# cosmicBboy/movenet

Measured on AMD Instinct MI355X. Metric: autoregressive audio samples/sec (16 kHz, 30-layer WaveNet, whole job), higher is better.
Workload: dtype f32

## Files before the change

movenet_amd/csrc/generate_fold.hip:

```cpp
#include <cstdlib>
#include <type_traits>

#include "common.h"
#include "gen_common.h"
#include "pipe_common.h"

namespace mvn {

namespace fold {
constexpr int C = 64, Q = 256, NT = 512, LPS = 3;
constexpr int KQ = 4, KPER = 16, NF4 = 4;
constexpr int MAT_F = 2 * C * C;
enum { M_A0 = 0, M_A0P, M_A1, M_A2, M_B2P,
       M_B1, M_B1P, M_B2, M_RR, M_RS,
       M_WP0, M_WP1, M_WP2, M_SS,
       N_MAT };
constexpr int N_LDS_MAT = 4;
constexpr int V_CB1 = 0, V_CB2 = 2 * C, V_BSP = 4 * C, V_BR0 = 5 * C, V_BS0 = 6 * C, V_BR1 = 7 * C,
              V_BS1 = 8 * C, V_BR2 = 9 * C, VEC_F = 10 * C;
constexpr int STAGE_F = N_MAT * MAT_F + VEC_F;
constexpr int CTX_LAYER_F = MAT_F + 2 * C;
constexpr int EMB_F = 2 * Q * C;
constexpr int W1_F = Q * C, W2_F = Q * Q, WSL_F = C * C;
constexpr int HEAD_F = W1_F + Q + W2_F + Q + WSL_F + C;
// ... 15 lines not shown
    m.w[2 * i + 1] = v2f{v.z, v.w};
  }
}
__device__ __forceinline__ v2f pk_fma_hi(v2f w, v2f xpair, v2f acc) {
  asm("v_pk_fma_f32 %0, %1, %2, %0 op_sel:[0,1,0]" : "+v"(acc) : "v"(w), "v"(xpair));
  return acc;
}
__device__ __forceinline__ v2f pk_mul_hi(v2f w, v2f xpair) {
  v2f r;
  asm("v_pk_mul_f32 %0, %1, %2 op_sel:[0,1]" : "=v"(r) : "v"(w), "v"(xpair));
  return r;
}
template <bool INIT>
__device__ __forceinline__ void pair_acc(v2f (&acc)[4], const v2f (&w)[16], const f4 (&x)[4]) {
#pragma unroll
  for (int i = 0; i < 4; ++i) {
    if (INIT && i == 0) {
      acc[0] = w[0] * v2f{x[0].x, x[0].x};
      acc[1] = w[1] * v2f{x[0].y, x[0].y};
      acc[2] = w[2] * v2f{x[0].z, x[0].z};
      acc[3] = pk_mul_hi(w[3], v2f{x[0].z, x[0].w});
    } else {
      acc[0] = __builtin_elementwise_fma(w[4 * i], v2f{x[i].x, x[i].x}, acc[0]);
      acc[1] = __builtin_elementwise_fma(w[4 * i + 1], v2f{x[i].y, x[i].y}, acc[1]);
      acc[2] = __builtin_elementwise_fma(w[4 * i + 2], v2f{x[i].z, x[i].z}, acc[2]);
      acc[3] = pk_fma_hi(w[4 * i + 3], v2f{x[i].z, x[i].w}, acc[3]);
    }
  }
}
__device__ __forceinline__ v2f pair_sum(const v2f (&acc)[4]) { return (acc[0] + acc[2]) + (acc[1] + acc[3]); }
template <int H>
__device__ __forceinline__ float split_dot(const v2f (&w)[16], const f4 (&x)[4]) {
  v2f a0 = w[8 * H] * v2f{x[0].x, x[0].y}, a1 = w[8 * H + 1] * v2f{x[0].z, x[0].w};
  v2f a2 = w[8 * H + 2] * v2f{x[1].x, x[1].y}, a3 = w[8 * H + 3] * v2f{x[1].z, x[1].w};
  a0 = __builtin_elementwise_fma(w[8 * H + 4], v2f{x[2].x, x[2].y}, a0);
  a1 = __builtin_elementwise_fma(w[8 * H + 5], v2f{x[2].z, x[2].w}, a1);
  a2 = __builtin_elementwise_fma(w[8 * H + 6], v2f{x[3].x, x[3].y}, a2);
  a3 = __builtin_elementwise_fma(w[8 * H + 7], v2f{x[3].z, x[3].w}, a3);
  const v2f t = (a0 + a2) + (a1 + a3);
  return t.x + t.y;
}

typedef __attribute__((address_space(3))) float lds_f;
typedef float vf4 __attribute__((ext_vector_type(4)));
typedef __attribute__((address_space(3))) vf4 lds_f4;
__device__ __forceinline__ f4 lds_load4(unsigned addr) {
  const vf4 v = *(const lds_f4 *)(uintptr_t)addr;
  f4 r;
  r.x = v.x; r.y = v.y; r.z = v.z; r.w = v.w;
  return r;
}
__device__ __forceinline__ unsigned lds_addr(const float *p) { return (unsigned)(uintptr_t)(lds_f *)p; }
#define LDSF(addr, off) (*(lds_f *)(uintptr_t)((addr) + 4u * (unsigned)(off)))
template <int N4>
__device__ __forceinline__ void ldsv(f4 (&x)[N4], unsigned addr, int off) {
#pragma unroll
  for (int i = 0; i < N4; ++i) x[i] = lds_load4(addr + 4u * (unsigned)off + 16u * i);
}

__device__ __forceinline__ v2f pair_dot_lds(unsigned waddr, unsigned xaddr) {
  v2f acc[4];
#pragma unroll
  for (int i = 0; i < 4; ++i) {
    const f4 wa = lds_load4(waddr + 4096u * (2 * i)), wb = lds_load4(waddr + 4096u * (2 * i + 1));
    const f4 x = lds_load4(xaddr + 16u * i);
    if (i == 0) {
      acc[0] = v2f{wa.x, wa.y} * v2f{x.x, x.x};
      acc[1] = v2f{wa.z, wa.w} * v2f{x.y, x.y};
      acc[2] = v2f{wb.x, wb.y} * v2f{x.z, x.z};
      acc[3] = pk_mul_hi(v2f{wb.z, wb.w}, v2f{x.z, x.w});
    } else {
      acc[0] = __builtin_elementwise_fma(v2f{wa.x, wa.y}, v2f{x.x, x.x}, acc[0]);
      acc[1] = __builtin_elementwise_fma(v2f{wa.z, wa.w}, v2f{x.y, x.y}, acc[1]);
      acc[2] = __builtin_elementwise_fma(v2f{wb.x, wb.y}, v2f{x.z, x.z}, acc[2]);
      acc[3] = pk_fma_hi(v2f{wb.z, wb.w}, v2f{x.z, x.w}, acc[3]);
    }
  }
  return pair_sum(acc);
}
template <int H>
__device__ __forceinline__ float split_dot_lds(unsigned waddr, unsigned xaddr) {
  f4 w[4], x[4];
#pragma unroll
  for (int i = 0; i < 4; ++i) {
    w[i] = lds_load4(waddr + 4096u * (4 * H + i));
    x[i] = lds_load4(xaddr + 16u * i);
  }
  v2f a0 = v2f{w[0].x, w[0].y} * v2f{x[0].x, x[0].y}, a1 = v2f{w[0].z, w[0].w} * v2f{x[0].z, x[0].w};
  v2f a2 = v2f{w[1].x, w[1].y} * v2f{x[1].x, x[1].y}, a3 = v2f{w[1].z, w[1].w} * v2f{x[1].z, x[1].w};
  a0 = __builtin_elementwise_fma(v2f{w[2].x, w[2].y}, v2f{x[2].x, x[2].y}, a0);
  a1 = __builtin_elementwise_fma(v2f{w[2].z, w[2].w}, v2f{x[2].z, x[2].w}, a1);
  a2 = __builtin_elementwise_fma(v2f{w[3].x, w[3].y}, v2f{x[3].x, x[3].y}, a2);
  a3 = __builtin_elementwise_fma(v2f{w[3].z, w[3].w}, v2f{x[3].z, x[3].w}, a3);
  const v2f t = (a0 + a2) + (a1 + a3);
  return t.x + t.y;
}

template <bool MULTI>
__global__ __launch_bounds__(512, 2) void gen_fold_kernel(GenArgs a, u64 *hand, unsigned *err, int NS, int nb, int nseq) {
  using namespace fold;
  extern __shared__ __attribute__((aligned(16))) float smem[];
  const int tid = threadIdx.x, lane = tid & 63, wave = tid >> 6;
  const int xcd = blockIdx.x & 7, slot = blockIdx.x >> 3;
  const int in_xcd = (PIPE_XCD_CUS / NS) * NS;
  int b, s;
  if (slot < in_xcd) {
    b = xcd + 8 * (slot / NS);
    s = slot % NS;
  } else {
    const int idx = xcd * (PIPE_XCD_CUS - in_xcd) + (slot - in_xcd);
    b = 8 * (PIPE_XCD_CUS / NS) + idx / NS;
    s = idx % NS;
  }
  if (b >= nb) return;
  if (__hip_atomic_load(err, __ATOMIC_RELAXED, __HIP_MEMORY_SCOPE_AGENT) != 0) return;
  const int L = a.L;
  const int s_next = s + 1 == NS ? 0 : s + 1;
  const int G = MULTI ? (nseq - b + nb - 1) / nb : 1;
  int bq = b;
  u64 *inbox = hand + ((size_t)b * NS + s) * GRAN;
  u64 *outbox = hand + ((size_t)b * NS + s_next) * GRAN;
  int *iflag = (int *)(smem + LDS_FLOATS - 16);
  float *pfs = smem + LDS_FLOATS;
  const bool fast_edge = pipe_edge_is_fast(err + 16, b, s, s_next, NS, iflag);

  auto layer_stage = [&](auto first_stage) {
    constexpr bool FIRST = decltype(first_stage)::value;
    const bool last = s == NS - 2;
    const int l0 = s * LPS, nl = min(LPS, L - l0);
    const bool chain = tid < 256;
    const int t = tid & 255, c = t >> 2, kq = t & 3;
    const bool lead = kq == 0;
    float *lmat = smem;
    constexpr int O_XP = 0;
    constexpr int O_ZL = C;
    constexpr int O_Z0 = 2 * C, O_Z1 = 3 * C;
    constexpr int O_X0 = 4 * C;
    constexpr int O_B1 = 5 * C, O_B2 = 7 * C;
    constexpr int O_PAST = 9 * C;
    constexpr int O_CTX = 12 * C;
    constexpr int O_VEC = 13 * C;
    float *vec = smem + N_LDS_MAT * MAT_F;
    unsigned vc = lds_addr(vec) + 4u * c;
    unsigned vq = lds_addr(vec) + 4u * KPER * kq;
    asm volatile("" : "+v"(vc), "+v"(vq));
    u64 *ob = outbox + c;
    const u64 *ibs = inbox + 2 * C + c;
    float *ring = a.state + (size_t)b * a.state_per_seq;
    auto bind = [&](int g) {
      bq = b + g * nb;
      inbox = hand + ((size_t)bq * NS + s) * GRAN;
      outbox = hand + ((size_t)bq * NS + s_next) * GRAN;
      ob = outbox + c;
      ibs = inbox + 2 * C + c;
      ring = a.state + (size_t)bq * a.state_per_seq;
    };
    const float *sec = a.w + EMB_F + (size_t)s * STAGE_F;
    const float *vecs = sec + N_MAT * MAT_F;

    FoldMat m0, m1 = {}, m2, m3, m4;
    {
      const int first = chain ? M_A0 : M_B1;
      fold_load(m0, sec + (size_t)(first + 0) * MAT_F, t);
      if (!FIRST) fold_load(m1, sec + (size_t)(first + 1) * MAT_F, t);
      fold_load(m2, sec + (size_t)(first + 2) * MAT_F, t);
      fold_load(m3, sec + (size_t)(first + 3) * MAT_F, t);
      fold_load(m4, sec + (size_t)(first + 4) * MAT_F, t);
      const f4 *src = (const f4 *)(sec + (size_t)M_WP0 * MAT_F);
      for (int i = tid; i < N_LDS_MAT * MAT_F / 4; i += NT) ((f4 *)lmat)[i] = src[i];
    }
    float pf[LPS], pg[LPS];
    float (&xs)[LPS] = pf;
    int doff[LPS], dmask[LPS];
    for (int i = tid; i < VEC_F; i += NT) vec[O_VEC + i] = vecs[i];
#pragma unroll
    for (int j = 0; j < LPS; ++j) {
      pf[j] = 0.f; pg[j] = 0.f;
      const int l = l0 + j;
      dmask[j] = j < nl ? (1 << (l % a.layer_size)) - 1 : 0;
      doff[j] = j < nl ? ring_offset(l, a.layer_size, C) : 0;
    }

    float popv[LPS] = {0.f, 0.f, 0.f};
    auto prefetch_pops = [&](int tn) {
      if (MULTI && !chain && lead) {
        int cq = c;
        asm volatile("" : "+v"(cq));
#pragma unroll
        for (int j = 0; j < LPS; ++j)
          if (j < nl) popv[j] = ring_load(ring + doff[j] + cq + (tn & dmask[j]) * C);
      }
    };
    auto precompute = [&](int tn, bool push, bool popped) {
      int tq = t;
      asm volatile("" : "+v"(tq));
      const int cq = tq >> 2, kk = tq & 3;
      if (!chain && lead) {
#pragma unroll
        for (int j = 0; j < LPS; ++j)
          if (j < nl) {
            float *base = ring + doff[j] + cq;
            if (push) base[((tn - 1) & dmask[j]) * C] = xs[j];
            const float pv = (push && dmask[j] == 0) ? xs[j]
                             : (MULTI && popped) ? popv[j] : ring_load(base + (tn & dmask[j]) * C);
            vec[O_PAST + j * C + cq] = pv;
          }
      }
      if (a.ctx_tm && chain && tq < C) vec[O_CTX + tq] = a.ctx_tm[(size_t)bq * a.ctx_stride_b + (size_t)tn * C + tq];
      __syncthreads();
      if (chain) {
        const unsigned wm = lds_addr(lmat) + 16u * tq, xq = lds_addr(vec) + 4u * (O_PAST + KPER * kk);
        const v2f p0 = pair_dot_lds(wm, xq);
        const v2f p1 = pair_dot_lds(wm + 4u * MAT_F, xq + 4u * C);
        const v2f p2 = pair_dot_lds(wm + 8u * MAT_F, xq + 8u * C);
        pf[0] = chan_sum<KQ>(p0.x);
        pg[0] = chan_sum<KQ>(p0.y);
        pf[1] = chan_sum<KQ>(p1.x) + vec[O_VEC + V_CB1 + cq];
        pg[1] = chan_sum<KQ>(p1.y) + vec[O_VEC + V_CB1 + C + cq];
        pf[2] = chan_sum<KQ>(p2.x) + vec[O_VEC + V_CB2 + cq];
        pg[2] = chan_sum<KQ>(p2.y) + vec[O_VEC + V_CB2 + C + cq];
        if (a.ctx_tm) {
#pragma unroll
          for (int j = 0; j < LPS; ++j)
            if (j < nl) {
              const float *wc = a.wctx + (size_t)(l0 + j) * CTX_LAYER_F;
              pf[j] += chan_sum<KQ>(dot_stream<NF4>((const f4 *)wc, 256, tq, vec + O_CTX + KPER * kk)) + wc[MAT_F + cq];
              pg[j] += chan_sum<KQ>(dot_stream<NF4>((const f4 *)wc + NF4 * 256, 256, tq, vec + O_CTX + KPER * kk)) +
// ... 1 lines not shown
            }
        }
      }
    };
    auto save_pf = [&](int g) {
      if (MULTI && chain && lead) {
        float *q = pfs + ((size_t)g * C + c) * PFS_F;
        *(f4 *)q = f4{pf[0], pg[0], pf[1], pg[1]};
        *(v2f *)(q + 4) = v2f{pf[2], pg[2]};
      }
    };
    auto load_pf = [&](int g) {
      if (MULTI && chain) {
        const float *q = pfs + ((size_t)g * C + c) * PFS_F;
        const f4 v = *(const f4 *)q;
        const v2f w = *(const v2f *)(q + 4);
        pf[0] = v.x; pg[0] = v.y; pf[1] = v.z; pg[1] = v.w; pf[2] = w.x; pg[2] = w.y;
      }
    };
    __syncthreads();
    if (MULTI) {
      for (int g = 0; g < G; ++g) {
        bind(g);
        precompute(a.t_begin, false, false);
        save_pf(g);
        __syncthreads();
      }
    } else {
      precompute(a.t_begin, false, false);
    }

    bool alive = true;
    for (int ts = a.t_begin; ts < a.t_end && alive; ++ts)
    for (int g = 0; g < G; ++g) {
      if (MULTI) {
        bind(g);
        if (ts + 1 < a.t_end) prefetch_pops(ts + 1);
      }
      const unsigned epoch = (unsigned)(ts - a.t_begin + 1);
      if (wave == 0) {
        float v[2];
        const bool ok = FIRST ? wait_inbox64(inbox, epoch, err, v) : wait_inbox<2>(inbox, epoch, err, v);
        if (ok && (!FIRST || lane < 32)) {
          float *dst = vec + 2 * lane;
          dst[0] = v[0];
          dst[1] = v[1];
        }
        if (lane == 0) iflag[0] = ok ? 1 : 0;
      }
      lds_barrier();
      MVN_STAMP(b, s, ts - a.t_begin, 0);
      load_pf(g);
      float xv = 0.f;
      MVN_FINE(b, s, ts - a.t_begin, 0, 0);
      if (chain) {
        f4 xa[NF4], xb[NF4];
        ldsv<NF4>(xa, vq, O_XP);
        if (!FIRST) ldsv<NF4>(xb, vq, O_ZL);
        v2f acc[4];
        pair_acc<true>(acc, m0.w, xa);
        if (!FIRST) pair_acc<false>(acc, m1.w, xb);
        const v2f fg = pair_sum(acc);
        const float f = chan_sum<KQ>(fg.x) + pf[0];
        const float g = chan_sum<KQ>(fg.y) + pg[0];
        const float z = gate_fast(f, g);
        if (lead) LDSF(vc, O_Z0) = z;
        MVN_FINE(b, s, ts - a.t_begin, 1, 0);
      } else {
        f4 xa[NF4], xb[NF4];
        ldsv<NF4>(xa, vq, O_XP);
        if (!FIRST) ldsv<NF4>(xb, vq, O_ZL);
        v2f acc[4];
        pair_acc<true>(acc, m0.w, xa);
        if (!FIRST) pair_acc<false>(acc, m1.w, xb);
        const v2f fg = pair_sum(acc);
        float r = 0.f;
        if (!FIRST) r = split_dot<0>(m3.w, xb);
        const float f = chan_sum<KQ>(fg.x);
        const float g = chan_sum<KQ>(fg.y);
        if (!FIRST) r = chan_sum<KQ>(r);
        if (lead) {
          xv = LDSF(vc, O_XP) + r;
          LDSF(vc, O_X0) = xv;
          xs[0] = xv;
          LDSF(vc, O_B1) = f;
          LDSF(vc, O_B1 + C) = g;
        }
        MVN_FINE(b, s, ts - a.t_begin, 6, 256);
      }
      lds_barrier();
      MVN_FINE(b, s, ts - a.t_begin, 2, 0);
      v2f b2 = {0.f, 0.f};
      if (chain) {
        f4 xz[NF4];
        ldsv<NF4>(xz, vq, O_Z0);
        v2f acc[4], acc2[4];
        pair_acc<true>(acc, m2.w, xz);
        pair_acc<true>(acc2, m4.w, xz);
        const v2f fg = pair_sum(acc);
        b2 = pair_sum(acc2);
        asm volatile("" : "+v"(b2));
        const float f = chan_sum<KQ>(fg.x) + (LDSF(vc, O_B1) + pf[1]);
        const float g = chan_sum<KQ>(fg.y) + (LDSF(vc, O_B1 + C) + pg[1]);
        const float z = gate_fast(f, g);
        if (lead) LDSF(vc, O_Z1) = z;
        MVN_FINE(b, s, ts - a.t_begin, 3, 0);
      } else {
        f4 xa[NF4];
        ldsv<NF4>(xa, vq, O_X0);
        v2f acc[4];
        pair_acc<true>(acc, m2.w, xa);
        const v2f fg = pair_sum(acc);
        const float f = chan_sum<KQ>(fg.x);
        const float g = chan_sum<KQ>(fg.y);
        if (lead) {
          LDSF(vc, O_B2) = f;
          LDSF(vc, O_B2 + C) = g;
        }
        MVN_FINE(b, s, ts - a.t_begin, 7, 256);
      }
      lds_barrier();
      MVN_FINE(b, s, ts - a.t_begin, 4, 0);
      if (chain) {
        f4 xz[NF4];
        ldsv<NF4>(xz, vq, O_Z1);
        v2f acc[4];
        pair_acc<true>(acc, m3.w, xz);
        const v2f fg = pair_sum(acc) + b2;
        const float f = chan_sum<KQ>(fg.x) + (LDSF(vc, O_B2) + pf[2]);
        const float g = chan_sum<KQ>(fg.y) + (LDSF(vc, O_B2 + C) + pg[2]);
        const float z = gate_fast(f, g);
        if (lead) put_granule(ob + C, epoch, z, fast_edge);
        MVN_FINE(b, s, ts - a.t_begin, 5, 0);
      } else {
        u64 sk_peek = 0;
        if (!FIRST) sk_peek = peek_granule(ibs);
        f4 xz[NF4];
        ldsv<NF4>(xz, vq, O_Z1);
        auto stream = [&](bool send) {
          f4 xz0[NF4];
          ldsv<NF4>(xz0, vq, O_Z0);
          const float br0 = LDSF(vc, O_VEC + V_BR0), br1 = LDSF(vc, O_VEC + V_BR1), br2 = LDSF(vc, O_VEC + V_BR2);
          float r0 = split_dot<1>(m3.w, xz0);
          float r = split_dot<0>(m4.w, xz);
          r0 = chan_sum<KQ>(r0);
          r = chan_sum<KQ>(r);
          if (lead) {
            xv = (xv + br0) + r0;
            xs[1] = xv;
            xv = (xv + br1) + r;
            xs[2] = xv;
            if (send) put_granule(ob, epoch, xv + br2, fast_edge);
          }
          MVN_FINE(b, s, ts - a.t_begin, 8, 256);
        };
        auto skip = [&] {
          float k1 = split_dot<1>(m4.w, xz);
          unsigned wss = lds_addr(lmat + 3 * MAT_F) + 16u * t;
          asm volatile("" : "+v"(wss));
          float kp = 0.f;
          if (!FIRST) kp = split_dot_lds<0>(wss, vq + 4u * O_ZL);
          float k0 = split_dot_lds<1>(wss, vq + 4u * O_Z0);
          if (!FIRST) kp = chan_sum<KQ>(kp);
          k0 = chan_sum<KQ>(k0);
          k1 = chan_sum<KQ>(k1);
          if (lead) {
            const float bs0 = LDSF(vc, O_VEC + V_BS0), bs1 = LDSF(vc, O_VEC + V_BS1);
            float sk0 = 0.f;
            if (!FIRST) {
              const float bsp = LDSF(vc, O_VEC + V_BSP);
              const float skin = (unsigned)(sk_peek >> 32) == epoch ? __uint_as_float((unsigned)sk_peek)
                                                                    : wait_granule(ibs, epoch, err);
              sk0 = skin + (kp + bsp);
            }
            put_granule(ob + 2 * C, epoch, (sk0 + (k0 + bs0)) + (k1 + bs1), fast_edge);
          }
          MVN_FINE(b, s, ts - a.t_begin, 9, 256);
        };
        if (last) {
          skip();
          stream(false);
        } else {
          stream(true);
          skip();
        }
      }
      MVN_STAMP(b, s, ts - a.t_begin, 1);
      lds_barrier();
      if (iflag[0] == 0) {
        alive = false;
        break;
      }
      if (ts + 1 < a.t_end) {
        precompute(ts + 1, true, true);
        save_pf(g);
      } else if (!chain && lead) {
        int cq = c;
        asm volatile("" : "+v"(cq));
#pragma unroll
        for (int j = 0; j < LPS; ++j)
          if (j < nl) ring[doff[j] + cq + (ts & dmask[j]) * C] = xs[j];
      }
    }
  };
  if (s < NS - 1) {
    if (s == 0)
      layer_stage(std::true_type{});
    else
      layer_stage(std::false_type{});
    return;
  }

  {
    float *tab = smem;
    float *vec = smem + N_LDS_MAT * MAT_F;
    float *zlb = vec;
    float *a0 = zlb + C;
    float *a1 = a0 + C;
    float *lgb = a1 + Q;
    const float *E0 = tab, *E1 = tab + Q * C;
    const float *hw = a.w + EMB_F + (size_t)(NS - 1) * STAGE_F;
    const f4 *W1p = (const f4 *)hw, *W2p = (const f4 *)(hw + W1_F + Q);
    const float *b1 = hw + W1_F, *b2 = hw + W1_F + Q + W2_F;
    const f4 *WSp = (const f4 *)(hw + W1_F + Q + W2_F + Q);
    const float *bsl = hw + W1_F + Q + W2_F + Q + WSL_F;
    int *hidx = (int *)pfs;

    const int o1 = tid >> 1, q1 = tid & 1, og = tid >> 3, q2 = tid & 7;
    v2f wsl[4], w1[16], w2[4][16];
    {
      const f4 *src = (const f4 *)a.w;
      f4 *dst = (f4 *)tab;
      for (int i = tid; i < EMB_F / 4; i += NT) dst[i] = src[i];
      loadn<2>(wsl, WSp, NT, tid);
      loadn<8>(w1, W1p, NT, tid);
#pragma unroll
      for (int r = 0; r < 4; ++r) loadn<8>(w2[r], W2p + r * 8 * NT, NT, tid);
    }
    const float b1r = b1[o1];
    const float b2r = b2[4 * og + (q2 & 3)];
    const float bslr = bsl[og];
    __syncthreads();

    auto await = [&](const u64 *inbox, unsigned epoch) {
      float v[2];
      const bool ok = wait_inbox64(inbox + C, epoch, err, v);
      if (ok && lane < 32) {
        zlb[2 * lane] = v[0];
        zlb[2 * lane + 1] = v[1];
      }
      return ok;
    };
    auto logits = [&](const u64 *inbox, unsigned epoch, bool do_head) {
      MVN_FINE(b, NS - 1, epoch - 1, 0, 0);
      const u64 sk_peek = peek_granule(inbox + 2 * C + og);
      float sv = 0.f;
      if (do_head) {
        f4 x[2];
        ldsn<2>(x, zlb + 8 * q2);
        sv = dotn<2>(wsl, x);
        sv = quad_sum(sv);
        sv += other_quad(sv);
      }
      float skin = 0.f;
      if (q2 == 0)
        skin = (unsigned)(sk_peek >> 32) == epoch ? __uint_as_float((unsigned)sk_peek)
                                                  : wait_granule(inbox + 2 * C + og, epoch, err);
      MVN_FINE(b, NS - 1, epoch - 1, 1, 0);
      if (!do_head) return;
      if (q2 == 0) a0[og] = leaky(skin + (sv + bslr));
      lds_barrier();
      {
        f4 x[8];
        ldsn<8>(x, a0 + 32 * q1);
        float hsum = dotn<8>(w1, x);
        hsum += dpp_mov<DPP_XOR1>(hsum);
        if (q1 == 0) a1[o1] = leaky(hsum + b1r);
      }
      lds_barrier();
      MVN_FINE(b, NS - 1, epoch - 1, 3, 0);
      head_conv2_f32(w2, a1, lgb, og, q2, b2r);
      lds_barrier();
      MVN_FINE(b, NS - 1, epoch - 1, 4, 0);
    };
    head_loop<C, GRAN, MULTI, 2, 0>(a, hand, NS, nb, b, G, fast_edge, E0, E1, iflag, hidx, lgb, await, logits);
  }
}

struct FoldLayers {
  const float *fw[4], *gw[4], *rw[4], *rb[4], *sw[4], *sb[4];
};
__device__ __forceinline__ double fold_wc(const FoldLayers &p, int j, int row, int k) {
  return p.fw[j] ? (double)fg_elem(p.fw[j], p.gw[j], fold::C, row, fold::C + k) : 0.0;
}
__device__ __forceinline__ double fold_wr(const FoldLayers &p, int j, int o, int k) {
  return p.rw[j] ? (double)p.rw[j][(size_t)o * fold::C + k] : 0.0;
}
__device__ __forceinline__ double fold_br(const FoldLayers &p, int j, int o) { return p.rb[j] ? (double)p.rb[j][o] : 0.0; }

__global__ void pack_fold_stage_kernel(FoldLayers p, float *__restrict__ dst) {
  using namespace fold;
  const int i = blockIdx.x * blockDim.x + threadIdx.x;
  if (i >= STAGE_F) return;
  if (i >= N_MAT * MAT_F) {
    const int o = i - N_MAT * MAT_F;
    double v = 0.0;
    if (o < V_CB2) {
      for (int m = 0; m < C; ++m) v += fold_wc(p, 2, o - V_CB1, m) * fold_br(p, 1, m);
    } else if (o < V_BSP) {
      for (int m = 0; m < C; ++m) v += fold_wc(p, 3, o - V_CB2, m) * (fold_br(p, 1, m) + fold_br(p, 2, m));
    } else if (o < V_BR0) v = p.sb[0] ? p.sb[0][o - V_BSP] : 0.0;
    else if (o < V_BS0) v = fold_br(p, 1, o - V_BR0);
    else if (o < V_BR1) v = p.sb[1] ? p.sb[1][o - V_BS0] : 0.0;
    else if (o < V_BS1) v = fold_br(p, 2, o - V_BR1);
    else if (o < V_BR2) v = p.sb[2] ? p.sb[2][o - V_BS1] : 0.0;
    else v = fold_br(p, 3, o - V_BR2);
    dst[i] = (float)v;
    return;
  }
  const int mat = i / MAT_F, r = i - mat * MAT_F;
  const int e = r & 3, v4 = r >> 2, t = v4 & 255, i4 = v4 >> 8;
  const bool split = mat == M_RR || mat == M_RS || mat == M_SS;
  const int row = split ? (i4 / NF4) * C + t / KQ : (e & 1) * C + t / KQ;
  const int k = KPER * (t % KQ) + (split ? 4 * (i4 % NF4) + e : 2 * i4 + (e >> 1));
  double v = 0.0;
  auto prod = [&](int jc, int jr) {
    double acc = 0.0;
    for (int m = 0; m < C; ++m) acc += fold_wc(p, jc, row, m) * fold_wr(p, jr, m, k);
    return acc;
  };
  auto ws = [&](int j, int o) { return p.sw[j] ? (double)p.sw[j][(size_t)o * C + k] : 0.0; };
  auto wp = [&](int j) { return p.fw[j] ? (double)fg_elem(p.fw[j], p.gw[j], C, row, k) : 0.0; };
  switch (mat) {
    case M_A0: v = fold_wc(p, 1, row, k); break;
    case M_A0P: v = prod(1, 0); break;
    case M_A1: v = prod(2, 1); break;
    case M_A2: v = prod(3, 2); break;
    case M_B2P: v = prod(3, 1); break;
// ... 105 lines not shown
```

movenet_amd/csrc/pipe_common.h:

```cpp
#pragma once
#include <cstdio>
#include <cstdlib>
#include <cstring>

#include "common.h"
#include "gen_common.h"

namespace mvn {

typedef unsigned long long u64;
typedef float4 f4;

constexpr int PIPE_XCD_CUS = 32;
constexpr unsigned PIPE_SPIN_LIMIT = 1u << 23;
constexpr int HEAD_Q = 256, HEAD_NT = 512;

inline bool pipe_profiler_attached() {
  for (const char *v : {"ROCP_TOOL_LIBRARIES", "ROCPROFILER_REGISTER_FORCE_LOAD", "HSA_TOOLS_LIB", "ROCP_METRICS"})
    if (const char *e = getenv(v))
      if (e[0]) return true;
  if (const char *pre = getenv("LD_PRELOAD"))
    if (strstr(pre, "rocprof")) return true;
  bool found = false;
  if (FILE *f = fopen("/proc/self/maps", "r")) {
// ... 154 lines not shown
      typedef unsigned v2u __attribute__((ext_vector_type(2)));
      v2u g;
      asm volatile("global_load_dwordx2 %0, %1, off sc1\n\ts_waitcnt vmcnt(0)" : "=&v"(g) : "v"(p) : "memory");
      lo = g.x;
      hi = g.y;
    }
    if (hi == epoch) return __uint_as_float(lo);
    if ((spins & 255u) == 0) {
      const unsigned e = __hip_atomic_load(err, __ATOMIC_RELAXED, __HIP_MEMORY_SCOPE_AGENT);
      if (e != 0 || spins > PIPE_SPIN_LIMIT) {
        __hip_atomic_store(err, 1u, __ATOMIC_RELAXED, __HIP_MEMORY_SCOPE_AGENT);
        return __uint_as_float(lo);
      }
    }
    __builtin_amdgcn_s_sleep(1);
  }
}

template <int GL>
__device__ __forceinline__ bool wait_inbox(const u64 *in, unsigned epoch, unsigned *err,
                                           float (&v)[GL]) {
  static_assert(GL == 2 || GL == 4, "one or two 16-byte loads per lane");
  const int lane = threadIdx.x & 63;
  const u64 *p = in + 2 * lane;
  if (GL == 2) return wait16(p, epoch, err, v[0], v[1]);
  for (unsigned spins = 1;; ++spins) {
    v4u g0, g1;
    asm volatile("global_load_dwordx4 %0, %2, off sc1\n\t"
                 "global_load_dwordx4 %1, %2, off offset:1024 sc1\n\ts_waitcnt vmcnt(0)"
                 : "=&v"(g0), "=&v"(g1) : "v"(p) : "memory");
    const bool ok = g0.y == epoch && g0.w == epoch && g1.y == epoch && g1.w == epoch;
    if (__all(ok)) {
      v[0] = __uint_as_float(g0.x);
      v[1] = __uint_as_float(g0.z);
      v[GL - 2] = __uint_as_float(g1.x);
      v[GL - 1] = __uint_as_float(g1.z);
      return true;
    }
    if ((spins & 255u) == 0) {
      const unsigned e = __hip_atomic_load(err, __ATOMIC_RELAXED, __HIP_MEMORY_SCOPE_AGENT);
      if (e != 0 || spins > PIPE_SPIN_LIMIT) {
        if (lane == 0) __hip_atomic_store(err, 1u, __ATOMIC_RELAXED, __HIP_MEMORY_SCOPE_AGENT);
        return false;
      }
    }
    __builtin_amdgcn_s_sleep(1);
  }
}

__device__ __forceinline__ bool wait_inbox64(const u64 *in, unsigned epoch, unsigned *err, float (&v)[2]) {
  return wait16(in + 2 * (threadIdx.x & 31), epoch, err, v[0], v[1]);
}

template <int CTRL>
__device__ __forceinline__ float dpp_mov(float v) {
  return __int_as_float(__builtin_amdgcn_update_dpp(0, __float_as_int(v), CTRL, 0xF, 0xF, true));
}
constexpr int DPP_XOR1 = 0xB1;
constexpr int DPP_XOR2 = 0x4E;
constexpr int DPP_HALF_MIRROR = 0x141;
constexpr int DPP_MIRROR = 0x140;

__device__ __forceinline__ float quad_sum(float v) {
  v += dpp_mov<DPP_XOR1>(v);
  v += dpp_mov<DPP_XOR2>(v);
  return v;
}
__device__ __forceinline__ float other_quad(float v) { return dpp_mov<DPP_HALF_MIRROR>(v); }

__device__ __forceinline__ float lane_value(float v, int lane) {
  return __int_as_float(__builtin_amdgcn_readlane(__float_as_int(v), lane));
}
__device__ __forceinline__ float wave_sum_dpp(float v) {
  v = quad_sum(v);
  v += dpp_mov<DPP_HALF_MIRROR>(v);
  v += dpp_mov<DPP_MIRROR>(v);
  return (lane_value(v, 0) + lane_value(v, 16)) + (lane_value(v, 32) + lane_value(v, 48));
}
__device__ __forceinline__ float wave_max_dpp(float v) {
  v = fmaxf(v, dpp_mov<DPP_XOR1>(v));
  v = fmaxf(v, dpp_mov<DPP_XOR2>(v));
  v = fmaxf(v, dpp_mov<DPP_HALF_MIRROR>(v));
  v = fmaxf(v, dpp_mov<DPP_MIRROR>(v));
  return fmaxf(fmaxf(lane_value(v, 0), lane_value(v, 16)), fmaxf(lane_value(v, 32), lane_value(v, 48)));
}

__device__ __forceinline__ float gate_fast(float f, float g) {
  const float a = __expf(-2.0f * fabsf(f));
  const float e = __expf(-g);
  const float num = copysignf(1.0f - a, f);
  const float den = (1.0f + a) * (1.0f + e);
  return num * __builtin_amdgcn_rcpf(den);
}

__device__ __forceinline__ void argmax_take(float &bv, int &bi, float ov, int oi) {
  if (ov > bv || (ov == bv && oi < bi)) {
    bv = ov;
    bi = oi;
  }
}
template <int CTRL>
__device__ __forceinline__ int dpp_movi(int v) {
  return __builtin_amdgcn_update_dpp(0, v, CTRL, 0xF, 0xF, true);
}


// ... 184 lines not shown
    incl += dpp_mov<0x112>(incl);
    incl += dpp_mov<0x114>(incl);
    incl += dpp_mov<0x118>(incl);
    {
      const float r0 = lane_value(incl, 15), r1 = lane_value(incl, 31), r2 = lane_value(incl, 47);
      const int row = lane >> 4;
      incl += row == 0 ? 0.f : row == 1 ? r0 : row == 2 ? r0 + r1 : (r0 + r1) + r2;
    }
    const float total = lane_value(incl, 63);
    const float target = uniform * total;
    const float cdf = incl - lsum;
    int cand = Q - 1;
    bool hit = false;
#pragma unroll
    for (int k = 3; k >= 0; --k) {
      const float c_k = cdf + (k == 0 ? p[0] : k == 1 ? p[0] + p[1]
                                              : k == 2 ? (p[0] + p[1]) + p[2]
                                                       : ((p[0] + p[1]) + p[2]) + p[3]);
      if (c_k > target) {
        cand = 4 * lane + k;
        hit = true;
      }
    }
    const unsigned long long lanes = __builtin_amdgcn_ballot_w64(hit);
    pick = lanes ? __builtin_amdgcn_readlane(cand, __builtin_ctzll(lanes)) : Q - 1;
  } else {
    float bv = p[0];
    int bi = 4 * lane;
#pragma unroll
    for (int k = 1; k < 4; ++k)
      if (p[k] > bv) {
        bv = p[k];
        bi = 4 * lane + k;
      }
    argmax_take(bv, bi, dpp_mov<DPP_XOR1>(bv), dpp_movi<DPP_XOR1>(bi));
    argmax_take(bv, bi, dpp_mov<DPP_XOR2>(bv), dpp_movi<DPP_XOR2>(bi));
    argmax_take(bv, bi, dpp_mov<DPP_HALF_MIRROR>(bv), dpp_movi<DPP_HALF_MIRROR>(bi));
    argmax_take(bv, bi, dpp_mov<DPP_MIRROR>(bv), dpp_movi<DPP_MIRROR>(bi));
    float rv = lane_value(bv, 0);
    pick = __builtin_amdgcn_readlane(bi, 0);
#pragma unroll
    for (int row = 16; row < 64; row += 16)
      argmax_take(rv, pick, lane_value(bv, row), __builtin_amdgcn_readlane(bi, row));
  }
  return pick;
}

__device__ __forceinline__ void head_conv2_f32(const v2f (&w2)[4][16], const float *a1, float *lgb, int og, int q2,
                                               float b2r) {
  f4 x[8];
  ldsn<8>(x, a1 + 32 * q2);
  float s0 = dotn<8>(w2[0], x), s1 = dotn<8>(w2[1], x);
  float s2 = dotn<8>(w2[2], x), s3 = dotn<8>(w2[3], x);
  s0 = quad_sum(s0); s0 += other_quad(s0);
  s1 = quad_sum(s1); s1 += other_quad(s1);
  s2 = quad_sum(s2); s2 += other_quad(s2);
  s3 = quad_sum(s3); s3 += other_quad(s3);
  const int sel = q2 & 3;
  if (q2 < 4) lgb[4 * og + sel] = (sel == 0 ? s0 : sel == 1 ? s1 : sel == 2 ? s2 : s3) + b2r;
}

template <int C, int GRAN, bool MULTI, int NZ, int NZ_SENT = NZ, class Await, class Logits>
__device__ __forceinline__ void head_loop(const GenArgs &a, u64 *hand, int NS, int nb, int b, int G, bool fast_edge,
                                          const float *E0, const float *E1, int *iflag, int *hidx, const float *lgb,
                                          Await await, Logits logits) {
  static_assert(GRAN == (1 + NZ) * C && NZ_SENT <= NZ, "residual stream + NZ zero lanes");
  const int lane = threadIdx.x & 63, wave = threadIdx.x >> 6, s = NS - 1;
  int bq;
  const u64 *inbox;
  u64 *outbox;
  int32_t *samples;
  auto bind = [&](int g) {
    bq = b + g * nb;
    inbox = hand + ((size_t)bq * NS + s) * GRAN;
    outbox = hand + (size_t)bq * NS * GRAN;
    samples = a.samples + (size_t)bq * a.stride;
  };
  int idx_cur = 0, idx_prev = -1;
  auto send_h0 = [&](unsigned ep) {
    const int ic = min(max(idx_cur, 0), a.Q - 1), ip = min(idx_prev, a.Q - 1);
#pragma unroll
    for (int j = 0; j < C / 64; ++j) {
      const int ch = lane + 64 * j;
      float v = E1[ic * C + ch];
      if (ip >= 0) v += E0[ip * C + ch];
      put_granule(outbox + ch, ep, v, fast_edge);
#pragma unroll
      for (int z = 1; z <= NZ_SENT; ++z) put_granule(outbox + z * C + ch, ep, 0.f, fast_edge);
    }
  };
  for (int g = 0; g < G; ++g) {
    bind(g);
    if (wave == 0) {
      idx_cur = samples[a.t_begin];
      idx_prev = a.t_begin > 0 ? samples[a.t_begin - 1] : -1;
      if (a.t_begin < a.t_end) send_h0(1u);
      MVN_STAMP(b, s, 0, 1);
      if (MULTI && lane == 0) {
        hidx[2 * g] = idx_cur;
        hidx[2 * g + 1] = idx_prev;
      }
    }
  }
  if (MULTI) __syncthreads();

  for (int ts = a.t_begin; ts < a.t_end; ++ts)
  for (int g = 0; g < G; ++g) {
    if (MULTI) {
      bind(g);
      if (wave == 0) {
        idx_cur = hidx[2 * g];
        idx_prev = hidx[2 * g + 1];
      }
    }
    const unsigned epoch = (unsigned)(ts - a.t_begin + 1);
    const int u = ts + 1;
    const bool want_out = (a.logits_out || a.choices_out) && u >= a.logits_t0;
    const bool do_head = u < a.n_total && (u >= a.n_given || want_out);
    int next_idx = 0;
    float uni = 0.f;
    if (wave == 0 && a.temperature > 0.f) {
      uni = philox_uniform(a.seed, (uint32_t)u, (uint32_t)bq);
      asm volatile("" : "+v"(uni));
    }
    if (wave == 0) {
      if (u < a.n_given) next_idx = samples[u];
      const bool ok = await(inbox, epoch);
      if (lane == 0) iflag[0] = ok ? 1 : 0;
    }
    lds_barrier();
    MVN_STAMP(b, s, ts - a.t_begin, 0);
    logits(inbox, epoch, do_head);
    if (wave == 0) {
      int pick = 0;
      if (do_head) {
        const f4 lv = ((const f4 *)lgb)[lane];
        const float lg[4] = {lv.x, lv.y, lv.z, lv.w};
        if (a.logits_out && u >= a.logits_t0 && 4 * lane < a.Q)
          ((f4 *)(a.logits_out + ((size_t)bq * (a.n_total - a.logits_t0) + (u - a.logits_t0)) * a.Q))[lane] = lv;
        pick = choose_class(lg, a.temperature, uni, lane, a.Q);
        if (u >= a.n_given) next_idx = pick;
      }
      idx_prev = idx_cur;
      idx_cur = next_idx;
      if (ts + 1 < a.t_end) send_h0(epoch + 1);
      MVN_STAMP(b, s, ts + 1 - a.t_begin, 1);
      MVN_FINE(b, s, ts - a.t_begin, 5, 0);
      if (do_head && lane == 0) {
        if (a.choices_out && u >= a.logits_t0) a.choices_out[(size_t)bq * a.n_total + u] = pick;
        if (u >= a.n_given) samples[u] = pick;
      }
      if (MULTI && lane == 0) {
        hidx[2 * g] = idx_cur;
        hidx[2 * g + 1] = idx_prev;
      }
    }
    if (iflag[0] == 0) return;
  }
}

__device__ __forceinline__ bool pack_head_f32(int i, int C, int W1N, int qm, const float *w1, const float *b1,
                                              const float *w2, const float *b2, float *__restrict__ dst) {
  constexpr int Q = HEAD_Q, NT = HEAD_NT;
  const int W1_F = Q * C, W2_F = Q * Q;
  if (i < W1_F) {
    const int e = i & 3, v = i >> 2, tid = v & (NT - 1), i4 = v >> 9;
    const int o = tid >> 1;
    dst[i] = o < qm ? w1[(size_t)o * C + W1N * (tid & 1) + 4 * i4 + e] : 0.f;
  } else if (i < W1_F + Q) {
    dst[i] = i - W1_F < qm ? b1[i - W1_F] : 0.f;
  } else if (i < W1_F + Q + W2_F) {
    const int ii = i - W1_F - Q;
    const int e = ii & 3, v = ii >> 2, tid = v & (NT - 1), rest = v >> 9, r = rest >> 3, i8 = rest & 7;
    const int o = 4 * (tid >> 3) + r, k = 32 * (tid & 7) + 4 * i8 + e;
    dst[i] = (o < qm && k < qm) ? w2[(size_t)o * qm + k] : 0.f;
  } else if (i < W1_F + Q + W2_F + Q) {
    const int o = i - W1_F - Q - W2_F;
    dst[i] = o < qm ? b2[o] : -INFINITY;
  } else {
    return false;
  }
  return true;
// ... 4 lines not shown
```

Measured before the change: 1.113 million.

## Hoist skip-path dots into earlier phases and merge head skip receive into inbox

```diff
diff --git a/movenet_amd/csrc/generate_fold.hip b/movenet_amd/csrc/generate_fold.hip
--- a/movenet_amd/csrc/generate_fold.hip
+++ b/movenet_amd/csrc/generate_fold.hip
@@ -118,13 +118,10 @@
   return pair_sum(acc);
 }
 template <int H>
-__device__ __forceinline__ float split_dot_lds(unsigned waddr, unsigned xaddr) {
-  f4 w[4], x[4];
-#pragma unroll
-  for (int i = 0; i < 4; ++i) {
-    w[i] = lds_load4(waddr + 4096u * (4 * H + i));
-    x[i] = lds_load4(xaddr + 16u * i);
-  }
+__device__ __forceinline__ float split_dot_lds(unsigned waddr, const f4 (&x)[4]) {
+  f4 w[4];
+#pragma unroll
+  for (int i = 0; i < 4; ++i) w[i] = lds_load4(waddr + 4096u * (4 * H + i));
   v2f a0 = v2f{w[0].x, w[0].y} * v2f{x[0].x, x[0].y}, a1 = v2f{w[0].z, w[0].w} * v2f{x[0].z, x[0].w};
   v2f a2 = v2f{w[1].x, w[1].y} * v2f{x[1].x, x[1].y}, a3 = v2f{w[1].z, w[1].w} * v2f{x[1].z, x[1].w};
   a0 = __builtin_elementwise_fma(v2f{w[2].x, w[2].y}, v2f{x[2].x, x[2].y}, a0);
@@ -319,6 +316,9 @@
       MVN_STAMP(b, s, ts - a.t_begin, 0);
       load_pf(g);
       float xv = 0.f;
+      float r0p = 0.f;
+      float kp = 0.f;
+      float part = 0.f;
       MVN_FINE(b, s, ts - a.t_begin, 0, 0);
       if (chain) {
         f4 xa[NF4], xb[NF4];
@@ -353,6 +353,12 @@
           LDSF(vc, O_B1) = f;
           LDSF(vc, O_B1 + C) = g;
         }
+        if (!FIRST) {
+          __builtin_amdgcn_sched_barrier(0);
+          unsigned wss = lds_addr(lmat + 3 * MAT_F) + 16u * t;
+          asm volatile("" : "+v"(wss));
+          kp = chan_sum<KQ>(split_dot_lds<0>(wss, xb));
+        }
         MVN_FINE(b, s, ts - a.t_begin, 6, 256);
       }
       lds_barrier();
@@ -375,6 +381,10 @@
       } else {
         f4 xa[NF4];
         ldsv<NF4>(xa, vq, O_X0);
+        u64 sk_peek = 0;
+        if (!FIRST) sk_peek = peek_granule(ibs);
+        f4 xz0[NF4];
+        ldsv<NF4>(xz0, vq, O_Z0);
         v2f acc[4];
         pair_acc<true>(acc, m2.w, xa);
         const v2f fg = pair_sum(acc);
@@ -383,6 +393,24 @@
         if (lead) {
           LDSF(vc, O_B2) = f;
           LDSF(vc, O_B2 + C) = g;
+        }
+        __builtin_amdgcn_sched_barrier(0);
+        r0p = split_dot<1>(m3.w, xz0);
+        {
+          unsigned wss = lds_addr(lmat + 3 * MAT_F) + 16u * t;
+          asm volatile("" : "+v"(wss));
+          const float k0 = chan_sum<KQ>(split_dot_lds<1>(wss, xz0));
+          if (lead) {
+            const float bs0 = LDSF(vc, O_VEC + V_BS0);
+            float sk0 = 0.f;
+            if (!FIRST) {
+              const float bsp = LDSF(vc, O_VEC + V_BSP);
+              const float skin = (unsigned)(sk_peek >> 32) == epoch ? __uint_as_float((unsigned)sk_peek)
+                                                                    : wait_granule(ibs, epoch, err);
+              sk0 = skin + (kp + bsp);
+            }
+            part = sk0 + (k0 + bs0);
+          }
         }
         MVN_FINE(b, s, ts - a.t_begin, 7, 256);
       }
@@ -400,15 +428,11 @@
         if (lead) put_granule(ob + C, epoch, z, fast_edge);
         MVN_FINE(b, s, ts - a.t_begin, 5, 0);
       } else {
-        u64 sk_peek = 0;
-        if (!FIRST) sk_peek = peek_granule(ibs);
         f4 xz[NF4];
         ldsv<NF4>(xz, vq, O_Z1);
         auto stream = [&](bool send) {
-          f4 xz0[NF4];
-          ldsv<NF4>(xz0, vq, O_Z0);
           const float br0 = LDSF(vc, O_VEC + V_BR0), br1 = LDSF(vc, O_VEC + V_BR1), br2 = LDSF(vc, O_VEC + V_BR2);
-          float r0 = split_dot<1>(m3.w, xz0);
+          float r0 = r0p;
           float r = split_dot<0>(m4.w, xz);
           r0 = chan_sum<KQ>(r0);
           r = chan_sum<KQ>(r);
@@ -423,25 +447,8 @@
         };
         auto skip = [&] {
           float k1 = split_dot<1>(m4.w, xz);
-          unsigned wss = lds_addr(lmat + 3 * MAT_F) + 16u * t;
-          asm volatile("" : "+v"(wss));
-          float kp = 0.f;
-          if (!FIRST) kp = split_dot_lds<0>(wss, vq + 4u * O_ZL);
-          float k0 = split_dot_lds<1>(wss, vq + 4u * O_Z0);
-          if (!FIRST) kp = chan_sum<KQ>(kp);
-          k0 = chan_sum<KQ>(k0);
           k1 = chan_sum<KQ>(k1);
-          if (lead) {
-            const float bs0 = LDSF(vc, O_VEC + V_BS0), bs1 = LDSF(vc, O_VEC + V_BS1);
-            float sk0 = 0.f;
-            if (!FIRST) {
-              const float bsp = LDSF(vc, O_VEC + V_BSP);
-              const float skin = (unsigned)(sk_peek >> 32) == epoch ? __uint_as_float((unsigned)sk_peek)
-                                                                    : wait_granule(ibs, epoch, err);
-              sk0 = skin + (kp + bsp);
-            }
-            put_granule(ob + 2 * C, epoch, (sk0 + (k0 + bs0)) + (k1 + bs1), fast_edge);
-          }
+          if (lead) put_granule(ob + 2 * C, epoch, part + (k1 + LDSF(vc, O_VEC + V_BS1)), fast_edge);
           MVN_FINE(b, s, ts - a.t_begin, 9, 256);
         };
         if (last) {
@@ -482,7 +489,8 @@
     float *tab = smem;
     float *vec = smem + N_LDS_MAT * MAT_F;
     float *zlb = vec;
-    float *a0 = zlb + C;
+    float *skb = zlb + C;
+    float *a0 = skb + C;
     float *a1 = a0 + C;
     float *lgb = a1 + Q;
     const float *E0 = tab, *E1 = tab + Q * C;
@@ -511,8 +519,8 @@
 
     auto await = [&](const u64 *inbox, unsigned epoch) {
       float v[2];
-      const bool ok = wait_inbox64(inbox + C, epoch, err, v);
-      if (ok && lane < 32) {
+      const bool ok = wait_inbox<2>(inbox + C, epoch, err, v);
+      if (ok) {
         zlb[2 * lane] = v[0];
         zlb[2 * lane + 1] = v[1];
       }
@@ -520,7 +528,7 @@
     };
     auto logits = [&](const u64 *inbox, unsigned epoch, bool do_head) {
       MVN_FINE(b, NS - 1, epoch - 1, 0, 0);
-      const u64 sk_peek = peek_granule(inbox + 2 * C + og);
+      if (!do_head) return;
       float sv = 0.f;
       if (do_head) {
         f4 x[2];
@@ -530,11 +538,8 @@
         sv += other_quad(sv);
       }
       float skin = 0.f;
-      if (q2 == 0)
-        skin = (unsigned)(sk_peek >> 32) == epoch ? __uint_as_float((unsigned)sk_peek)
-                                                  : wait_granule(inbox + 2 * C + og, epoch, err);
+      if (q2 == 0) skin = skb[og];
       MVN_FINE(b, NS - 1, epoch - 1, 1, 0);
-      if (!do_head) return;
       if (q2 == 0) a0[og] = leaky(skin + (sv + bslr));
       lds_barrier();
       {
```

New measurement: 990,400. -11.0%, worse.

## Replace mid-step workgroup barrier with LDS epoch flags between chain and side waves

Applied to the files above, without the earlier changes.

```diff
diff --git a/movenet_amd/csrc/generate_fold.hip b/movenet_amd/csrc/generate_fold.hip
--- a/movenet_amd/csrc/generate_fold.hip
+++ b/movenet_amd/csrc/generate_fold.hip
@@ -91,10 +91,20 @@
 }
 __device__ __forceinline__ unsigned lds_addr(const float *p) { return (unsigned)(uintptr_t)(lds_f *)p; }
 #define LDSF(addr, off) (*(lds_f *)(uintptr_t)((addr) + 4u * (unsigned)(off)))
+#define LDSF_ORDERED(addr, off) (*(volatile lds_f *)(uintptr_t)((addr) + 4u * (unsigned)(off)))
 template <int N4>
 __device__ __forceinline__ void ldsv(f4 (&x)[N4], unsigned addr, int off) {
 #pragma unroll
   for (int i = 0; i < N4; ++i) x[i] = lds_load4(addr + 4u * (unsigned)off + 16u * i);
+}
+
+template <int N4>
+__device__ __forceinline__ void ldsv_ordered(f4 (&x)[N4], unsigned addr, int off) {
+#pragma unroll
+  for (int i = 0; i < N4; ++i) {
+    const vf4 v = *(volatile const lds_f4 *)(uintptr_t)(addr + 4u * (unsigned)off + 16u * i);
+    x[i].x = v.x; x[i].y = v.y; x[i].z = v.z; x[i].w = v.w;
+  }
 }
 
 __device__ __forceinline__ v2f pair_dot_lds(unsigned waddr, unsigned xaddr) {
@@ -212,6 +222,8 @@
     float (&xs)[LPS] = pf;
     int doff[LPS], dmask[LPS];
     for (int i = tid; i < VEC_F; i += NT) vec[O_VEC + i] = vecs[i];
+    if (!MULTI && tid < 8) iflag[8 + tid] = 0;
+    const unsigned jw = lds_addr((const float *)(iflag + 8));
 #pragma unroll
     for (int j = 0; j < LPS; ++j) {
       pf[j] = 0.f; pg[j] = 0.f;
@@ -333,6 +345,7 @@
         const float z = gate_fast(f, g);
         if (lead) LDSF(vc, O_Z0) = z;
         MVN_FINE(b, s, ts - a.t_begin, 1, 0);
+        if (!MULTI) joint_arrive(jw + 4u * wave, epoch);
       } else {
         f4 xa[NF4], xb[NF4];
         ldsv<NF4>(xa, vq, O_XP);
@@ -354,27 +367,63 @@
           LDSF(vc, O_B1 + C) = g;
         }
         MVN_FINE(b, s, ts - a.t_begin, 6, 256);
-      }
-      lds_barrier();
-      MVN_FINE(b, s, ts - a.t_begin, 2, 0);
+        if (!MULTI) joint_arrive(jw + 4u * wave, epoch);
+      }
+      if (MULTI) lds_barrier();
+      unsigned spins = 0;
       v2f b2 = {0.f, 0.f};
       if (chain) {
         f4 xz[NF4];
-        ldsv<NF4>(xz, vq, O_Z0);
+        for (;;) {
+          if (MULTI) {
+            ldsv<NF4>(xz, vq, O_Z0);
+            break;
+          }
+          const v4u w = joint_peek(jw);
+          ldsv_ordered<NF4>(xz, vq, O_Z0);
+          if (joint_reached(w, epoch) || joint_give_up(spins, err, iflag)) break;
+        }
+        MVN_FINE(b, s, ts - a.t_begin, 2, 0);
         v2f acc[4], acc2[4];
         pair_acc<true>(acc, m2.w, xz);
+        v4u hw = {epoch, epoch, epoch, epoch};
+        float b1f, b1g;
+        if (MULTI) {
+          b1f = LDSF(vc, O_B1);
+          b1g = LDSF(vc, O_B1 + C);
+        } else {
+          __builtin_amdgcn_sched_barrier(0);
+          hw = joint_peek(jw + 16u);
+          b1f = LDSF_ORDERED(vc, O_B1);
+          b1g = LDSF_ORDERED(vc, O_B1 + C);
+          __builtin_amdgcn_sched_barrier(0);
+        }
         pair_acc<true>(acc2, m4.w, xz);
         const v2f fg = pair_sum(acc);
         b2 = pair_sum(acc2);
         asm volatile("" : "+v"(b2));
-        const float f = chan_sum<KQ>(fg.x) + (LDSF(vc, O_B1) + pf[1]);
-        const float g = chan_sum<KQ>(fg.y) + (LDSF(vc, O_B1 + C) + pg[1]);
+        while (!MULTI && !joint_reached(hw, epoch) && !joint_give_up(spins, err, iflag)) {
+          hw = joint_peek(jw + 16u);
+          b1f = LDSF_ORDERED(vc, O_B1);
+          b1g = LDSF_ORDERED(vc, O_B1 + C);
+        }
+        const float f = chan_sum<KQ>(fg.x) + (b1f + pf[1]);
+        const float g = chan_sum<KQ>(fg.y) + (b1g + pg[1]);
         const float z = gate_fast(f, g);
         if (lead) LDSF(vc, O_Z1) = z;
         MVN_FINE(b, s, ts - a.t_begin, 3, 0);
       } else {
         f4 xa[NF4];
-        ldsv<NF4>(xa, vq, O_X0);
+        for (;;) {
+          if (MULTI) {
+            ldsv<NF4>(xa, vq, O_X0);
+            break;
+          }
+          const v4u w = joint_peek(jw + 16u);
+          ldsv_ordered<NF4>(xa, vq, O_X0);
+          if (joint_reached(w, epoch) || joint_give_up(spins, err, iflag)) break;
+        }
+        MVN_FINE(b, s, ts - a.t_begin, 10, 256);
         v2f acc[4];
         pair_acc<true>(acc, m2.w, xa);
         const v2f fg = pair_sum(acc);
diff --git a/movenet_amd/csrc/pipe_common.h b/movenet_amd/csrc/pipe_common.h
--- a/movenet_amd/csrc/pipe_common.h
+++ b/movenet_amd/csrc/pipe_common.h
@@ -230,6 +230,31 @@
   return wait16(in + 2 * (threadIdx.x & 31), epoch, err, v[0], v[1]);
 }
 
+typedef __attribute__((address_space(3))) unsigned lds_u32;
+typedef __attribute__((address_space(3))) v4u lds_v4u;
+constexpr unsigned JOINT_SPIN_LIMIT = 1u << 20;
+
+__device__ __forceinline__ void joint_arrive(unsigned word_addr, unsigned turn) {
+  asm volatile("" ::: "memory");
+  if ((threadIdx.x & 63) == 0)
+    __hip_atomic_store((lds_u32 *)(uintptr_t)word_addr, turn, __ATOMIC_RELAXED, __HIP_MEMORY_SCOPE_WORKGROUP);
+}
+__device__ __forceinline__ v4u joint_peek(unsigned words_addr) { return *(volatile lds_v4u *)(uintptr_t)words_addr; }
+__device__ __forceinline__ bool joint_reached(v4u w, unsigned turn) {
+  const unsigned m = min(min(w.x, w.y), min(w.z, w.w));
+  return (unsigned)__builtin_amdgcn_readfirstlane((int)m) >= turn;
+}
+__device__ __forceinline__ bool joint_give_up(unsigned &spins, unsigned *err, int *iflag) {
+  if ((++spins & 255u) != 0) return false;
+  const unsigned e = __hip_atomic_load(err, __ATOMIC_RELAXED, __HIP_MEMORY_SCOPE_AGENT);
+  if (e == 0 && spins < JOINT_SPIN_LIMIT) return false;
+  if ((threadIdx.x & 63) == 0) {
+    __hip_atomic_store(err, 1u, __ATOMIC_RELAXED, __HIP_MEMORY_SCOPE_AGENT);
+    iflag[0] = 0;
+  }
+  return true;
+}
+
 template <int CTRL>
 __device__ __forceinline__ float dpp_mov(float v) {
   return __int_as_float(__builtin_amdgcn_update_dpp(0, __float_as_int(v), CTRL, 0xF, 0xF, true));
```

Result: slower. 1.113 million before, 1.049 million after (-5.7%).

## Hoist skip and residual dot products earlier and overlap head skip wait

Applied to the files above, without the earlier changes.

```diff
diff --git a/movenet_amd/csrc/generate_fold.hip b/movenet_amd/csrc/generate_fold.hip
--- a/movenet_amd/csrc/generate_fold.hip
+++ b/movenet_amd/csrc/generate_fold.hip
@@ -125,6 +125,21 @@
     w[i] = lds_load4(waddr + 4096u * (4 * H + i));
     x[i] = lds_load4(xaddr + 16u * i);
   }
+  v2f a0 = v2f{w[0].x, w[0].y} * v2f{x[0].x, x[0].y}, a1 = v2f{w[0].z, w[0].w} * v2f{x[0].z, x[0].w};
+  v2f a2 = v2f{w[1].x, w[1].y} * v2f{x[1].x, x[1].y}, a3 = v2f{w[1].z, w[1].w} * v2f{x[1].z, x[1].w};
+  a0 = __builtin_elementwise_fma(v2f{w[2].x, w[2].y}, v2f{x[2].x, x[2].y}, a0);
+  a1 = __builtin_elementwise_fma(v2f{w[2].z, w[2].w}, v2f{x[2].z, x[2].w}, a1);
+  a2 = __builtin_elementwise_fma(v2f{w[3].x, w[3].y}, v2f{x[3].x, x[3].y}, a2);
+  a3 = __builtin_elementwise_fma(v2f{w[3].z, w[3].w}, v2f{x[3].z, x[3].w}, a3);
+  const v2f t = (a0 + a2) + (a1 + a3);
+  return t.x + t.y;
+}
+
+template <int H>
+__device__ __forceinline__ float split_dot_ldsw(unsigned waddr, const f4 (&x)[4]) {
+  f4 w[4];
+#pragma unroll
+  for (int i = 0; i < 4; ++i) w[i] = lds_load4(waddr + 4096u * (4 * H + i));
   v2f a0 = v2f{w[0].x, w[0].y} * v2f{x[0].x, x[0].y}, a1 = v2f{w[0].z, w[0].w} * v2f{x[0].z, x[0].w};
   v2f a2 = v2f{w[1].x, w[1].y} * v2f{x[1].x, x[1].y}, a3 = v2f{w[1].z, w[1].w} * v2f{x[1].z, x[1].w};
   a0 = __builtin_elementwise_fma(v2f{w[2].x, w[2].y}, v2f{x[2].x, x[2].y}, a0);
@@ -210,6 +225,7 @@
     }
     float pf[LPS], pg[LPS];
     float (&xs)[LPS] = pf;
+    float &r0p = pg[0], &skp = pg[1];
     int doff[LPS], dmask[LPS];
     for (int i = tid; i < VEC_F; i += NT) vec[O_VEC + i] = vecs[i];
 #pragma unroll
@@ -373,16 +389,41 @@
         if (lead) LDSF(vc, O_Z1) = z;
         MVN_FINE(b, s, ts - a.t_begin, 3, 0);
       } else {
-        f4 xa[NF4];
+        u64 sk_peek = 0;
+        if (!FIRST && last) sk_peek = peek_granule(ibs);
+        f4 xa[NF4], xz0[NF4];
         ldsv<NF4>(xa, vq, O_X0);
+        ldsv<NF4>(xz0, vq, O_Z0);
         v2f acc[4];
         pair_acc<true>(acc, m2.w, xa);
+        r0p = split_dot<1>(m3.w, xz0);
+        asm volatile("" : "+v"(r0p));
         const v2f fg = pair_sum(acc);
         const float f = chan_sum<KQ>(fg.x);
         const float g = chan_sum<KQ>(fg.y);
         if (lead) {
           LDSF(vc, O_B2) = f;
           LDSF(vc, O_B2 + C) = g;
+        }
+        if (last) {
+          unsigned wss = lds_addr(lmat + 3 * MAT_F) + 16u * t;
+          asm volatile("" : "+v"(wss));
+          float k0 = split_dot_ldsw<1>(wss, xz0);
+          float kp = 0.f;
+          if (!FIRST) kp = split_dot_lds<0>(wss, vq + 4u * O_ZL);
+          if (!FIRST) kp = chan_sum<KQ>(kp);
+          k0 = chan_sum<KQ>(k0);
+          if (lead) {
+            const float bs0 = LDSF(vc, O_VEC + V_BS0);
+            float sk0 = 0.f;
+            if (!FIRST) {
+              const float bsp = LDSF(vc, O_VEC + V_BSP);
+              const float skin = (unsigned)(sk_peek >> 32) == epoch ? __uint_as_float((unsigned)sk_peek)
+                                                                    : wait_granule(ibs, epoch, err);
+              sk0 = skin + (kp + bsp);
+            }
+            skp = sk0 + (k0 + bs0);
+          }
         }
         MVN_FINE(b, s, ts - a.t_begin, 7, 256);
       }
@@ -401,16 +442,13 @@
         MVN_FINE(b, s, ts - a.t_begin, 5, 0);
       } else {
         u64 sk_peek = 0;
-        if (!FIRST) sk_peek = peek_granule(ibs);
+        if (!FIRST && !last) sk_peek = peek_granule(ibs);
         f4 xz[NF4];
         ldsv<NF4>(xz, vq, O_Z1);
         auto stream = [&](bool send) {
-          f4 xz0[NF4];
-          ldsv<NF4>(xz0, vq, O_Z0);
           const float br0 = LDSF(vc, O_VEC + V_BR0), br1 = LDSF(vc, O_VEC + V_BR1), br2 = LDSF(vc, O_VEC + V_BR2);
-          float r0 = split_dot<1>(m3.w, xz0);
+          float r0 = chan_sum<KQ>(r0p);
           float r = split_dot<0>(m4.w, xz);
-          r0 = chan_sum<KQ>(r0);
           r = chan_sum<KQ>(r);
           if (lead) {
             xv = (xv + br0) + r0;
@@ -445,7 +483,10 @@
           MVN_FINE(b, s, ts - a.t_begin, 9, 256);
         };
         if (last) {
-          skip();
+          float k1 = split_dot<1>(m4.w, xz);
+          k1 = chan_sum<KQ>(k1);
+          if (lead) put_granule(ob + 2 * C, epoch, skp + (k1 + LDSF(vc, O_VEC + V_BS1)), fast_edge);
+          MVN_FINE(b, s, ts - a.t_begin, 9, 256);
           stream(false);
         } else {
           stream(true);
@@ -492,6 +533,7 @@
     const f4 *WSp = (const f4 *)(hw + W1_F + Q + W2_F + Q);
     const float *bsl = hw + W1_F + Q + W2_F + Q + WSL_F;
     int *hidx = (int *)pfs;
+    float *skb = lgb + Q;
 
     const int o1 = tid >> 1, q1 = tid & 1, og = tid >> 3, q2 = tid & 7;
     v2f wsl[4], w1[16], w2[4][16];
@@ -518,9 +560,18 @@
       }
       return ok;
     };
+    float skin = 0.f;
+    auto await_skip = [&](const u64 *inbox, unsigned epoch) {
+      if (wave == 0) return;
+      const int ch = (wave == 1 && q2 >= 4) ? og - 8 : og;
+      float v0 = 0.f, v1 = 0.f;
+      wait16(inbox + 2 * C + (ch & ~1), epoch, err, v0, v1);
+      skin = (ch & 1) ? v1 : v0;
+      if (wave == 1 && q2 == 4) skb[ch] = skin;
+    };
     auto logits = [&](const u64 *inbox, unsigned epoch, bool do_head) {
       MVN_FINE(b, NS - 1, epoch - 1, 0, 0);
-      const u64 sk_peek = peek_granule(inbox + 2 * C + og);
+      if (wave == 0) skin = skb[og];
       float sv = 0.f;
       if (do_head) {
         f4 x[2];
@@ -529,10 +580,6 @@
         sv = quad_sum(sv);
         sv += other_quad(sv);
       }
-      float skin = 0.f;
-      if (q2 == 0)
-        skin = (unsigned)(sk_peek >> 32) == epoch ? __uint_as_float((unsigned)sk_peek)
-                                                  : wait_granule(inbox + 2 * C + og, epoch, err);
       MVN_FINE(b, NS - 1, epoch - 1, 1, 0);
       if (!do_head) return;
       if (q2 == 0) a0[og] = leaky(skin + (sv + bslr));
@@ -550,7 +597,7 @@
       lds_barrier();
       MVN_FINE(b, NS - 1, epoch - 1, 4, 0);
     };
-    head_loop<C, GRAN, MULTI, 2, 0>(a, hand, NS, nb, b, G, fast_edge, E0, E1, iflag, hidx, lgb, await, logits);
+    head_loop<C, GRAN, MULTI, 2, 0>(a, hand, NS, nb, b, G, fast_edge, E0, E1, iflag, hidx, lgb, await, logits, await_skip);
   }
 }
 
diff --git a/movenet_amd/csrc/pipe_common.h b/movenet_amd/csrc/pipe_common.h
--- a/movenet_amd/csrc/pipe_common.h
+++ b/movenet_amd/csrc/pipe_common.h
@@ -520,18 +520,24 @@
   ldsn<8>(x, a1 + 32 * q2);
   float s0 = dotn<8>(w2[0], x), s1 = dotn<8>(w2[1], x);
   float s2 = dotn<8>(w2[2], x), s3 = dotn<8>(w2[3], x);
-  s0 = quad_sum(s0); s0 += other_quad(s0);
-  s1 = quad_sum(s1); s1 += other_quad(s1);
-  s2 = quad_sum(s2); s2 += other_quad(s2);
-  s3 = quad_sum(s3); s3 += other_quad(s3);
-  const int sel = q2 & 3;
-  if (q2 < 4) lgb[4 * og + sel] = (sel == 0 ? s0 : sel == 1 ? s1 : sel == 2 ? s2 : s3) + b2r;
-}
-
-template <int C, int GRAN, bool MULTI, int NZ, int NZ_SENT = NZ, class Await, class Logits>
+  const int e = q2 < 4 ? q2 : 7 - q2;
+  const bool odd = (e & 1) != 0, upper = (e & 2) != 0;
+  float ka = odd ? s1 : s0, kb = odd ? s3 : s2;
+  ka += dpp_mov<DPP_XOR1>(odd ? s0 : s1);
+  kb += dpp_mov<DPP_XOR1>(odd ? s2 : s3);
+  float k = upper ? kb : ka;
+  k += dpp_mov<DPP_XOR2>(upper ? ka : kb);
+  k += other_quad(k);
+  if (q2 < 4) lgb[4 * og + q2] = k + b2r;
+}
+
+struct HeadNoHook {
+  __device__ __forceinline__ void operator()(const u64 *, unsigned) const {}
+};
+template <int C, int GRAN, bool MULTI, int NZ, int NZ_SENT = NZ, class Await, class Logits, class Hook = HeadNoHook>
 __device__ __forceinline__ void head_loop(const GenArgs &a, u64 *hand, int NS, int nb, int b, int G, bool fast_edge,
                                           const float *E0, const float *E1, int *iflag, int *hidx, const float *lgb,
-                                          Await await, Logits logits) {
+                                          Await await, Logits logits, Hook before_barrier = Hook()) {
   static_assert(GRAN == (1 + NZ) * C && NZ_SENT <= NZ, "residual stream + NZ zero lanes");
   const int lane = threadIdx.x & 63, wave = threadIdx.x >> 6, s = NS - 1;
   int bq;
@@ -545,13 +551,19 @@
     samples = a.samples + (size_t)bq * a.stride;
   };
   int idx_cur = 0, idx_prev = -1;
+  float e0[C / 64];
+  auto fetch_e0 = [&](int idx) {
+    const int ip = min(idx, a.Q - 1);
+#pragma unroll
+    for (int j = 0; j < C / 64; ++j) e0[j] = ip >= 0 ? E0[ip * C + lane + 64 * j] : 0.f;
+  };
   auto send_h0 = [&](unsigned ep) {
-    const int ic = min(max(idx_cur, 0), a.Q - 1), ip = min(idx_prev, a.Q - 1);
+    const int ic = min(max(idx_cur, 0), a.Q - 1);
 #pragma unroll
     for (int j = 0; j < C / 64; ++j) {
       const int ch = lane + 64 * j;
       float v = E1[ic * C + ch];
-      if (ip >= 0) v += E0[ip * C + ch];
+      if (idx_prev >= 0) v += e0[j];
       put_granule(outbox + ch, ep, v, fast_edge);
 #pragma unroll
       for (int z = 1; z <= NZ_SENT; ++z) put_granule(outbox + z * C + ch, ep, 0.f, fast_edge);
@@ -562,6 +574,7 @@
     if (wave == 0) {
       idx_cur = samples[a.t_begin];
       idx_prev = a.t_begin > 0 ? samples[a.t_begin - 1] : -1;
+      fetch_e0(idx_prev);
       if (a.t_begin < a.t_end) send_h0(1u);
       MVN_STAMP(b, s, 0, 1);
       if (MULTI && lane == 0) {
@@ -592,10 +605,12 @@
       asm volatile("" : "+v"(uni));
     }
     if (wave == 0) {
+      fetch_e0(idx_cur);
       if (u < a.n_given) next_idx = samples[u];
       const bool ok = await(inbox, epoch);
       if (lane == 0) iflag[0] = ok ? 1 : 0;
     }
+    before_barrier(inbox, epoch);
     lds_barrier();
     MVN_STAMP(b, s, ts - a.t_begin, 0);
     logits(inbox, epoch, do_head);
```

Result: slower. 1.111 million before, 1.079 million after (-2.9%).
